# tzjtatata/Myriad

Measured on AMD Instinct MI355X. Metric: images/sec fine-tune step (Vicuna-7B + LoRA-style adapters, 224px), higher is better.
Workload: dtype bf16

## Files before the change

include/myriad_hip.h:

```cpp
#ifndef MYRIAD_HIP_H
#define MYRIAD_HIP_H
#include <stdint.h>

#ifdef __cplusplus
extern "C" {
#endif

typedef struct ihipStream_t* mh_stream_t;

#define MH_OK 0
#define MH_ERR_ARG (-1)
#define MH_ERR_LAUNCH (-2)
#define MH_ERR_UNSUPPORTED (-3)

#define MH_GEMM_OUT_F32 1
#define MH_GEMM_GELU 2
#define MH_GEMM_REGSTAGE 4

int mh_gemm_bf16_nt(const void* A, int lda, const void* B, int ldb, void* C, int ldc, int M, int N, int K,
                    const float* bias, const float* residual, int ldr, int flags, float alpha, mh_stream_t s);

int mh_gemm_plan(int M, int N, int K, int flags, int* kernel, int* splits);

int mh_prof_start(int capacity, mh_stream_t s);
// ... 242 lines not shown
                                   const int* kv_len, const int* live, const float* cos_tab, const float* sin_tab, void* out,
                                   long ldo, float* partials, long partials_floats, int B, int H, int D, int T_cap, int chunk,
                                   float scale, mh_stream_t s);
int mh_patchify_nchw(const float* img, void* out, int B, int C, int H, int W, int P, int Kpad, mh_stream_t s);
int mh_scatter_rows_f32(const float* src, const int* rows, float* dst, long ldd, long n, int D, int accumulate,
                        mh_stream_t s);
int mh_cast_f32_to_bf16(const float* x, void* y, long n, mh_stream_t s);
int mh_cast_bf16_to_f32(const void* x, float* y, long n, mh_stream_t s);
int mh_transpose_to_bf16(const void* in, int in_is_f32, long ldi, void* out, long ldo, int R, int C, mh_stream_t s);
long mh_refresh_bf16_pair_desc_bytes(void);
long mh_refresh_bf16_pair_pack(void* host_table, int index, long first_tile, const float* src, void* dst, long ld_dst,
                               void* dst_t, long ld_t, int R, int C);
int mh_refresh_bf16_pair(const void* dev_table, int n_desc, long total_tiles, mh_stream_t s);
int mh_colsum_f32(const float* in, long ld, float* out, long R, int C, mh_stream_t s);
int mh_scale_f32(float* x, float a, long n, mh_stream_t s);

int mh_adamw_step(float* p, const float* g, float* m, float* v, void* shadow_bf16, long n, double lr, double beta1,
                  double beta2, double eps, double weight_decay, int step, double grad_scale, mh_stream_t s);

int mh_patch_blend_u8(void* out, const void* src, const void* masks, const void* ops, const int* hs, const int* ws,
                      int n_ops, int B, int H, int W, void* union_mask, const void* patches, mh_stream_t s);
int mh_patch_label(const void* dest, const void* out, const void* union_mask, void* sums_ws, void* lm_ws, float* label,
                   const double* factor, int B, int H, int W, int mode, int tol, double k, double x0, mh_stream_t s);
int mh_patch_resize_u8(const void* src, int image, int H, int W, int sy, int sx, int sh, int sw, const int* xi, const int* xw,
                       const int* yi, const int* yw, void* out, int h, int w, mh_stream_t s);
long mh_patch_poisson_ws_doubles(int h, int w);
int mh_patch_poisson_u8(void* out, int image, int H, int W, const void* patch, int hp, int wp, const void* pms,
                        const void* eroded, int y0s, int x0s, int dy0, int dx0, int h, int w, const double* Sh, const double* cy,
                        const double* Sw, const double* cx, double* ws, int mixed, mh_stream_t s);

int mh_adamw_gated(float* p, const float* g, float* m, float* v, long n, double lr, double beta1, double beta2, double eps,
                   double weight_decay, double grad_scale, const float* used, const int* steps, mh_stream_t s);
int mh_adamw_bump(const float* used, int* steps, int n, mh_stream_t s);

int mh_l2norm_rows(const float* x, long ldx, void* y_bf16, float* y_f32, long ldy, int M, int D, float eps, mh_stream_t s);
int mh_pair_logits(const float* p, long ldp, const float* text, float* out, long rows, int rows_per_batch, int C, float scale,
                   mh_stream_t s);
int mh_zs_accumulate(const float* logits, float* mask_acc, float* map_acc, int B, int h, int S, float w, mh_stream_t s);
int mh_rowmax_skip(const float* scores, long lds, float* acc, long rows, int cols, int period, float w, mh_stream_t s);
int mh_bilinear_ac(const float* in, float* out, int B, int h, int w, int H, int W, int one_minus, mh_stream_t s);

typedef struct mh_ctx mh_ctx;
int mh_ctx_create(mh_ctx** out);
int mh_ctx_destroy(mh_ctx* ctx);
int mh_ctx_set_workspace(mh_ctx* ctx, mh_stream_t stream, void* ptr, long bytes);
int mh_ctx_make_current(mh_ctx* ctx);
int mh_ctx_comm_id(void* id128);
int mh_ctx_comm_init(mh_ctx* ctx, const void* id128, int rank, int world);
int mh_ctx_world(const mh_ctx* ctx);
int mh_allreduce_start(mh_ctx* ctx, float* buf, long n, mh_stream_t producer);
#define MH_DT_F32 0
#define MH_DT_BF16 1
int mh_allreduce_start_dt(mh_ctx* ctx, void* buf, long n, int dt, mh_stream_t producer);
int mh_reduce_scatter_start(mh_ctx* ctx, const void* send, void* recv, long n_per_rank, int dt, mh_stream_t producer);
int mh_allgather_start(mh_ctx* ctx, const void* send, void* recv, long n_per_rank, int dt, mh_stream_t producer);
int mh_allreduce_wait(mh_ctx* ctx, mh_stream_t consumer);

const char* mh_version(void);
int mh_target_arch(void);

int mh_set_option(const char* name, int value);
int mh_get_option(const char* name);
int mh_bf16_round_check(const float* x, void* hw, void* hw_pk, void* sw, long n, mh_stream_t s);

int mh_image_resize_crop_norm(const void* img, int H, int W, long row_stride, const int* kh, const int* bh, int ksz_h,
                              const int* kv, const int* bv, int ksz_v, int crop_y0, int crop_x0, int out_h, int out_w, int y0,
// ... 8 lines not shown
```

myriad_amd/csrc/optim.hip:

```cpp
#include "common.h"

__global__ void adamw_kernel(float* __restrict__ p, const float* __restrict__ g, float* __restrict__ m,
                             float* __restrict__ v, bf16_t* __restrict__ shadow, long n4, float lr, float beta1,
                             float beta2, float omb1, float omb2, float eps, float wd, float bc1, float bc2_sqrt,
                             float gscale) {
  for (long it = blockIdx.x * (long)blockDim.x + threadIdx.x; it < n4; it += (long)gridDim.x * blockDim.x) {
    float4_t pp = *reinterpret_cast<const float4_t*>(p + it * 4);
    const float4_t gg = *reinterpret_cast<const float4_t*>(g + it * 4);
    float4_t mm = *reinterpret_cast<const float4_t*>(m + it * 4);
    float4_t vv = *reinterpret_cast<const float4_t*>(v + it * 4);
#pragma unroll
    for (int e = 0; e < 4; ++e) {
      const float gr = gg[e] * gscale;
      pp[e] *= (1.f - lr * wd);
      mm[e] = beta1 * mm[e] + omb1 * gr;
      vv[e] = beta2 * vv[e] + omb2 * gr * gr;
      const float denom = sqrtf(vv[e]) / bc2_sqrt + eps;
      pp[e] -= (lr / bc1) * (mm[e] / denom);
    }
    *reinterpret_cast<float4_t*>(p + it * 4) = pp;
    *reinterpret_cast<float4_t*>(m + it * 4) = mm;
    *reinterpret_cast<float4_t*>(v + it * 4) = vv;
    if (shadow) {
      uint2 pk;
      pk.x = pack_bf2(pp[0], pp[1]);
      pk.y = pack_bf2(pp[2], pp[3]);
      *reinterpret_cast<uint2*>(shadow + it * 4) = pk;
    }
  }
}

extern "C" int mh_adamw_step(float* p, const float* g, float* m, float* v, void* shadow_bf16, long n, double lr,
                             double beta1, double beta2, double eps, double weight_decay, int step, double grad_scale,
                             hipStream_t stream) {
  if (n <= 0) return MH_OK;
  if (n % 4 || step < 1) return MH_ERR_ARG;
  const float bc1 = (float)(1.0 - pow(beta1, (double)step));
  const float bc2s = (float)sqrt(1.0 - pow(beta2, (double)step));
  const float omb1 = (float)(1.0 - beta1), omb2 = (float)(1.0 - beta2);
  long grid = (n / 4 + 255) / 256;
  if (grid > 256 * 16) grid = 256 * 16;
  hipLaunchKernelGGL(adamw_kernel, dim3((int)grid), dim3(256), 0, stream, p, g, m, v, (bf16_t*)shadow_bf16, n / 4,
                     (float)lr, (float)beta1, (float)beta2, omb1, omb2, (float)eps, (float)weight_decay, bc1, bc2s,
                     (float)grad_scale);
  MH_CHECK_LAUNCH();
  return MH_OK;
}

__global__ void adamw_gated_kernel(float* __restrict__ p, const float* __restrict__ g, float* __restrict__ m,
                                   float* __restrict__ v, long n4, float lr, double beta1_d, double beta2_d, float eps,
                                   float wd, float gscale, const float* __restrict__ used, const int* __restrict__ steps) {
  if (*used <= 0.f) return;
  const double st = (double)(*steps + 1);
  const float bc1 = (float)(1.0 - pow(beta1_d, st));
  const float bc2_sqrt = (float)sqrt(1.0 - pow(beta2_d, st));
  const float omb1 = (float)(1.0 - beta1_d), omb2 = (float)(1.0 - beta2_d);
  const float beta1 = (float)beta1_d, beta2 = (float)beta2_d;
  for (long it = blockIdx.x * (long)blockDim.x + threadIdx.x; it < n4; it += (long)gridDim.x * blockDim.x) {
    float4_t pp = *reinterpret_cast<const float4_t*>(p + it * 4);
    const float4_t gg = *reinterpret_cast<const float4_t*>(g + it * 4);
    float4_t mm = *reinterpret_cast<const float4_t*>(m + it * 4);
    float4_t vv = *reinterpret_cast<const float4_t*>(v + it * 4);
#pragma unroll
    for (int e = 0; e < 4; ++e) {
      const float gr = gg[e] * gscale;
      pp[e] *= (1.f - lr * wd);
      mm[e] = beta1 * mm[e] + omb1 * gr;
      vv[e] = beta2 * vv[e] + omb2 * gr * gr;
      const float denom = sqrtf(vv[e]) / bc2_sqrt + eps;
      pp[e] -= (lr / bc1) * (mm[e] / denom);
    }
    *reinterpret_cast<float4_t*>(p + it * 4) = pp;
    *reinterpret_cast<float4_t*>(m + it * 4) = mm;
    *reinterpret_cast<float4_t*>(v + it * 4) = vv;
  }
}
__global__ void adamw_bump_kernel(const float* __restrict__ used, int* __restrict__ steps, int n) {
  const int i = blockIdx.x * blockDim.x + threadIdx.x;
  if (i < n && used[i] > 0.f) steps[i] += 1;
}

extern "C" int mh_adamw_gated(float* p, const float* g, float* m, float* v, long n, double lr, double beta1, double beta2,
                              double eps, double weight_decay, double grad_scale, const float* used, const int* steps,
                              hipStream_t stream) {
  if (n <= 0) return MH_OK;
  if (n % 4 || !used || !steps) return MH_ERR_ARG;
  long grid = (n / 4 + 255) / 256;
  if (grid > 256 * 16) grid = 256 * 16;
  hipLaunchKernelGGL(adamw_gated_kernel, dim3((int)grid), dim3(256), 0, stream, p, g, m, v, n / 4, (float)lr, beta1, beta2,
                     (float)eps, (float)weight_decay, (float)grad_scale, used, steps);
  MH_CHECK_LAUNCH();
  return MH_OK;
}
extern "C" int mh_adamw_bump(const float* used, int* steps, int n, hipStream_t stream) {
  if (n <= 0) return MH_OK;
  hipLaunchKernelGGL(adamw_bump_kernel, dim3((n + 63) / 64), dim3(64), 0, stream, used, steps, n);
  MH_CHECK_LAUNCH();
  return MH_OK;
}
```

myriad_amd/myriad.py:

```python
from __future__ import annotations

import numbers
import os
import random
from collections import OrderedDict
from typing import Dict, List, Optional, Tuple

import torch
import torch.nn as nn

from . import _lib, ops
from .eva_vit import EvaViTHIP
from .llama import LlamaHIP
from .networks import LoraAdaptor, VENet, from_reference_layout, to_reference_layout, ve_param_specs
from .qformer import QFormerHIP, qformer_param_specs
from .registry import registry

BF16, F32 = torch.bfloat16, torch.float32


def uses_weight_decay(name: str, ndim: int) -> bool:
    return not (ndim < 2 or "bias" in name or "ln" in name or "bn" in name)


# ... 67 lines not shown
            o, n = self.offsets[name]
            self.p[name] = self.flat_p[o:o + n].view(ishape)
            self.g[name] = self.flat_g[o:o + n].view(ishape)
            self.ref_shape[name] = rshape
        self.step = 0
        self.version = 0

    def n_params(self) -> int:
        return sum(n for _, n in self.offsets.values())

    def mark_used(self, used_modules) -> None:
        if not self.modules:
            return
        flags = torch.tensor([1.0 if m in used_modules else 0.0 for m in self.modules], dtype=F32)
        self.used.copy_(ops.h2d(flags, self.dev))

    def module_steps(self) -> Dict[str, int]:
        st = self.steps_dev.cpu().tolist()
        return {m: int(st[i]) for i, m in enumerate(self.modules)}

    def set_module_steps(self, steps: Dict[str, int]) -> None:
        host = torch.tensor([int(steps.get(m, 0)) for m in self.modules] or [0], dtype=torch.int32)
        self.steps_dev.copy_(host.to(self.dev))

    def module_range(self, module: str, decays: bool = True):
        if module not in self.modules:
            return None
        mi = self.modules.index(module)
        for m2, a, b, d in self.ranges:
            if m2 == mi and d == decays:
                return a, b
        return None

    def adamw_module(self, module: str, lr: float, weight_decay: float = 0.05, beta2: float = 0.999) -> None:
        mi = self.modules.index(module)
        self.version += 1
        for m2, a, b, decays in self.ranges:
            if m2 == mi:
                ops.adamw_gated(self.flat_p[a:b], self.flat_g[a:b], self.flat_m[a:b], self.flat_v[a:b], lr,
                                weight_decay if decays else 0.0, self.used[mi:mi + 1], self.steps_dev[mi:mi + 1], beta2=beta2)

    def adamw_pieces(self, pieces, lr: float, weight_decay: float = 0.05, beta2: float = 0.999, grad_scale: float = 1.0) -> None:
        self.version += 1
        for mi, a0, b0, decays in self.ranges:
            for lo, hi in pieces:
                a, b = max(a0, lo), min(b0, hi)
                if a < b:
                    ops.adamw_gated(self.flat_p[a:b], self.flat_g[a:b], self.flat_m[a:b], self.flat_v[a:b], lr,
                                    weight_decay if decays else 0.0, self.used[mi:mi + 1], self.steps_dev[mi:mi + 1], beta2=beta2,
                                    grad_scale=grad_scale)

    def adamw_step(self, lr: float, weight_decay: float = 0.05, beta2: float = 0.999, grad_scale: float = 1.0, shard=None,
                   skip=(), exclude=()):
        self.step += 1
        self.version += 1
        pieces = None
        if shard is not None:
            pieces = [tuple(shard)] if isinstance(shard[0], int) else [tuple(p) for p in shard]
            if sum(hi - lo for lo, hi in pieces) < self.total:
                self.moments_complete = False
        skip_idx = {self.modules.index(m) for m in skip if m in self.modules}
        for mi, a0, b0, decays in self.ranges:
            if mi in skip_idx:
                continue
            for lo, hi in (pieces if pieces is not None else [(a0, b0)]):
                a, b = max(a0, lo), min(b0, hi)
                if a >= b:
                    continue
                todo = [(a, b)]
                for ex_lo, ex_hi in exclude:
                    todo = [q for (x, y) in todo for q in ((x, min(y, ex_lo)), (max(x, ex_hi), y)) if q[0] < q[1]]
                for a, b in todo:
                    ops.adamw_gated(self.flat_p[a:b], self.flat_g[a:b], self.flat_m[a:b], self.flat_v[a:b], lr,
# ... 107 lines not shown
            if name in lora_init and name not in weights:
                src = lora_init[name]
            elif name in weights:
                src = weights[name]
            else:
                src = init_trainable(name, rshape)
            self.store.p[name].copy_(from_reference_layout(src.to(self._dev, F32), ishape))
            prm = nn.Parameter(self.store.p[name], requires_grad=True)
            prm.grad = self.store.g[name]
            self._params[name] = prm
            self._register_dotted(name, prm)
        if self.arch == "myriad":
            self.adaptor = LoraAdaptor(self.store.p, self.store.g)
            self.ve_tok = VENet("VETokenizer.", 5, self.Dl, self.store.p, self.store.g, self._dev)
            self.ve_ins = VENet("VEInstructor.", 1, self.Dq, self.store.p, self.store.g, self._dev)
        if self.use_lora:
            self.lora = LoraQV(len(self.llama.layers), self.Dl, int(cfg.get("lora_r", 8)),
                               float(cfg.get("lora_alpha", 16)), float(cfg.get("lora_dropout", 0.05)),
                               self.store.p, self.store.g, self._dev)
            self.lora.base_seed = int(cfg.get("lora_dropout_seed", torch.initial_seed())) & ((1 << 31) - 1)
            self.llama.attach_lora(self.lora)
        if self.train_qformer:
            self.query_tokens_f32 = self.store.p["query_tokens"]
            self.qformer.bind_trainable(self.store, need_denc=self.arch == "myriad" or self.train_vit)
        if self.train_vit:
            self.ln_w, self.ln_b = self.store.p["ln_vision.weight"], self.store.p["ln_vision.bias"]
            self.vit.bind_trainable(self.store, need_backward=need_bwd)
        self._pending_update = None
        self._vit_stream, self._vit_prefetched = None, None
        self._vit_graphs, self._vit_seen, self._vit_rest = {}, {}, None
        self._vit_split = int(os.environ.get("MYRIAD_VIT_SPLIT", "22"))
        self._vit_graph_on = os.environ.get("MYRIAD_VIT_GRAPH", "1") != "0"
        self._leaf_aside = os.environ.get("MYRIAD_LEAF_STREAM", "1") != "0"
        self._anchor = torch.zeros((), device=self._dev, requires_grad=True)
        self._ctx = None
        self._has_grads, self._bwd_gscale, self._bwd_prev = False, 1.0, None
        self._accum_count = 0
        self._bridge_used = set()

    def _register_dotted(self, name: str, prm: nn.Parameter):
        mod = self
        parts = name.split(".")
        for part in parts[:-1]:
            if not hasattr(mod, part) or not isinstance(getattr(mod, part), nn.Module):
                setattr(mod, part, nn.Module())
            mod = getattr(mod, part)
        mod.register_parameter(parts[-1], prm)

    @property
    def device(self):
        return self._dev

    def to(self, *args, **kwargs):
        dev = args[0] if args else kwargs.get("device", self._dev)
        if isinstance(dev, (str, torch.device)):
            d = torch.device(dev)
            if d.type != self._dev.type or (d.index is not None and d.index != self._dev.index):
                raise RuntimeError(f"{type(self).__name__} lives on {self._dev}; build it there (cfg.device; no CPU path exists)")
        return self

    def before_evaluation(self, **kwargs):
        pass

    def state_dict(self, *a, **k):
        self.finish_update()
        out = OrderedDict()
# ... 279 lines not shown
        self._acc_head = head
        fg = self.store.flat_g_comm
        if not accumulate:
            prev = None
        elif head is None:
            prev = fg.clone()
        else:
            prev = (fg[:head[0]].clone(), fg[head[1]:].clone())
        zeroed, self._g_zeroed = getattr(self, "_g_zeroed", None), None
        if zeroed is not None and not accumulate:
            torch.cuda.current_stream().wait_event(zeroed)
        elif head is None:
            fg.zero_()
        else:
            fg[:head[0]].zero_()
            fg[head[1]:].zero_()
        used = {"lora"} if self.use_lora else set()
        if self.arch == "myriad":
            used.add("expert_adaptor")
            if c["use_tok"]:
                used.add("VETokenizer")
            if c["use_ins"]:
                used.add("VEInstructor")
        else:
            used.add("llama_proj")
        if self.train_qformer:
            used.add("Qformer")
        if self.train_vit:
            used.update(("visual_encoder", "ln_vision"))
        self.store.mark_used(used)
        self._bridge_used = (self._bridge_used | used) if accumulate else set(used)
        self._bwd_gscale, self._bwd_prev = float(gscale), prev
        self._early_done = set()
        demb = self.llama.backward(defer_lora_join=True)
        self._prefetch_vit_rest()
        B, nq = c["B"], c["nq"]
        (c0, n0) = c["img_slices"][0]
        dimg = torch.empty((B, nq, self.Dl), dtype=F32, device=self._dev)
        ops.copy3d(demb[:, c0:c0 + n0], dimg)
        dimg_b = ops.to_bf16(dimg.view(B * nq, self.Dl))
        if self.arch != "myriad":
            ops.gemm_auto_f32(ops.transpose_to_bf16(dimg_b, 64), ops.transpose_to_bf16(c["qo_b"], 64),
                              self.store.g["llama_proj.weight"])
            self.store.g["llama_proj.bias"].copy_(ops.colsum(dimg.view(B * nq, self.Dl)))
            if self.train_qformer or self.train_vit:
                pwT = ops.transpose_to_bf16(ops.to_bf16(self.store.p["llama_proj.weight"]), 64)
                dqo = ops.gemm(dimg_b, pwT, out_dtype=F32).view(B, nq, self.Dq)
                dq, denc = self.qformer.backward(dqo, wgrads=self.train_qformer, want_denc=self.train_vit)
                if self.train_qformer:
                    self._query_tokens_grad(dq)
                if self.train_vit:
                    dy = self._ln_vision_backward(denc, c)
                    self.vit.backward(dy.view(B, c["N"], self.Dv), grads=self.vit.grad_views)
            if self.llama.lora is not None:
                self.llama.lora.join_wgrads()
            self._finish_backward()
            return
        dqo = ops.gemm(dimg_b, self.proj_wT, out_dtype=F32).view(B, nq, self.Dq)
        if c["use_tok"]:
            (cb, _), (ct, _) = c["img_slices"][1], c["img_slices"][2]
            dbase = torch.empty((B, 9, self.Dl), dtype=F32, device=self._dev)
            ops.copy3d(demb[:, cb:cb + 9], dbase)
            self.store.g["VETokenizer.base_prompts"].view(-1).copy_(ops.colsum(dbase.view(B, 9 * self.Dl)))
            dtok = torch.empty((B, 9, self.Dl), dtype=F32, device=self._dev)
            ops.copy3d(demb[:, ct:ct + 9], dtok)
            aux, main = (self._side_stream("leaf") if self._leaf_aside else torch.cuda.current_stream()), torch.cuda.current_stream()
            aux.wait_stream(main)
            leaf_keep = (dtok, self.ve_tok._saved)
            with torch.cuda.stream(aux):
                self.ve_tok.backward(dtok, accumulate_head=self._acc_head is not None)
                if early_adamw is not None and self._leaf_aside:
                    self.store.adamw_module("VETokenizer", *early_adamw)
                    self._early_done = {"VETokenizer"}
                if early_exchange is not None:
                    self._start_early_exchange(early_exchange)
                leaf_ev = torch.cuda.Event()
                leaf_ev.record()
        else:
            leaf_ev, leaf_keep = None, None
            if early_exchange is not None:
                self._start_early_exchange(early_exchange)
        dq, denc = self.qformer.backward(dqo, wgrads=self.train_qformer)
        if self.train_qformer:
            self._query_tokens_grad(dq)
        ins_ev, ins_keep = None, None
        if c["use_ins"]:
            dins = torch.empty((B, 49, self.Dq), dtype=F32, device=self._dev)
            ops.copy3d(dq[:, self.nq0:], dins)
            if self._leaf_aside and self._dev.type == "cuda" and os.environ.get("MYRIAD_INS_ASIDE", "1") != "0":
                aux, main = self._side_stream("leaf"), torch.cuda.current_stream()
                aux.wait_stream(main)
                ins_keep = (dins, self.ve_ins._saved)
                with torch.cuda.stream(aux):
                    self.ve_ins.backward(dins)
                    ins_ev = torch.cuda.Event()
                    ins_ev.record()
            else:
                self.ve_ins.backward(dins)
        dy = self._ln_vision_backward(denc, c)
        dx = self.adaptor.backward(dy, need_dx=self.train_vit)
        if self.train_vit:
            self.vit.backward(dx.view(B, c["N"], self.Dv), grads=self.vit.grad_views)
        if self.llama.lora is not None:
            self.llama.lora.join_wgrads()
        if leaf_ev is not None:
            torch.cuda.current_stream().wait_event(leaf_ev)
# ... 134 lines not shown
    def _take_prefetched_vit(self, samples):
        if self._vit_rest is not None and self._vit_rest[0] is samples:
            self._prefetch_vit_rest()
        if self._vit_prefetched is None or self._vit_prefetched[0] is not samples:
            return None
        _, out, ev = self._vit_prefetched
        self._vit_prefetched = None
        main = torch.cuda.current_stream()
        main.wait_event(ev)
        out.record_stream(main)
        return out

    def train_step(self, samples, lr: float, weight_decay: float = 0.05, allreduce=None, world: int = 1, dp=None,
                   overlap: bool = True, next_samples=None, accum_grad_iters: int = 1, accum_index=None, beta2: float = 0.999):
        with torch.no_grad():
            vit_out = self._take_prefetched_vit(samples)
            if next_samples is not None:
                self.prefetch_vit(next_samples)
            if self._pending_update is not None and vit_out is not None:
                self.finish_update()
            elif self._pending_update is not None and self.train_vit:
                self.finish_update()
            elif self._pending_update is not None:
                vit_out = self.vit.forward(self._image_of(samples))
                self.finish_update()
            if (self._accum_count == 0 and self._leaf_aside and self._dev.type == "cuda"
                    and os.environ.get("MYRIAD_EARLY_ZERO", "1") != "0"):
                aux, main = self._side_stream("leaf"), torch.cuda.current_stream()
                aux.wait_stream(main)
                with torch.cuda.stream(aux):
                    self.store.flat_g_comm.zero_()
                    self._g_zeroed = torch.cuda.Event()
                    self._g_zeroed.record(aux)
            try:
                loss = self._forward_impl(samples, True, vit_out=vit_out)
            except Exception:
                self._g_zeroed = None
                raise
            accumulate = self._accum_count > 0
            due = accum_update_due(self._accum_count + 1, accum_grad_iters, accum_index)
            early = (lr, weight_decay, beta2) if (due and not accumulate and (dp is None or dp.world == 1) and allreduce is None
                                                  and world == 1 and os.environ.get("MYRIAD_EARLY_ADAMW", "1") != "0") else None
            if dp is not None and dp.world > 1 and self.arch == "myriad" and hasattr(dp, "set_segments"):
                self._dp_segment(dp)
            early_x = None
            if (dp is not None and dp.world > 1 and overlap and due and not accumulate and self.arch == "myriad"
                    and hasattr(dp, "start_part") and os.environ.get("MYRIAD_DP_EARLY", "1") != "0"):
                k = self._dp_segment(dp)
                if k is not None:
                    early_x = (dp, k, (lr, weight_decay, beta2)) if os.environ.get("MYRIAD_DP_EARLY_ADAMW", "1") != "0" else (dp, k)
            self.backward(accumulate=accumulate, early_adamw=early, early_exchange=early_x)
            self._accum_count += 1
            if not due:
                return loss
            self._accum_count = 0
            if dp is not None and dp.world > 1 and overlap:
                dp.start(self.store.flat_g_comm, self.store.total)
                self._pending_update = (dp, lr, weight_decay, beta2)
            else:
                shard = None
                if dp is not None and dp.world > 1:
                    dp.allreduce(self.store.flat_g_comm, self.store.total)
                    shard = self._dp_shards(dp)
                elif allreduce is not None:
                    allreduce(self.store.flat_g_comm)
                    world = max(world, 1)
                self.store.adamw_step(lr, weight_decay, beta2=beta2, grad_scale=1.0 / (dp.world if dp is not None else world),
                                      shard=shard, skip=self._early_done)
                if shard is not None:
                    dp.gather_params(self.store.flat_p)
        return loss

    def _dp_shards(self, dp):
        if getattr(dp, "mode", "allreduce") != "rs_ag":
            return None
        return dp.shards(self.store.total) if hasattr(dp, "shards") else [dp.shard(self.store.total)[:2]]

    def _dp_segment(self, dp):
        if getattr(self, "_dp_seg_of", None) is not None and self._dp_seg_of[0] is dp:
            return self._dp_seg_of[1]
        k = None
        rng = self.store.module_range("VETokenizer", True)
        if rng is not None:
            a, b = ops.round_up(rng[0], 32), rng[1] // 32 * 32
            if b - a >= (1 << 20):
                dp.set_segments(self.store.total, [a, b])
                segs = dp.segments(self.store.total)
                k = segs.index((a, b)) if (a, b) in segs else None
        self._dp_seg_of = (dp, k)
        return k

    def finish_update(self):
        if self._pending_update is not None:
            dp, lr, wd, beta2 = self._pending_update
            self._pending_update = None
            if dp is None:
                self.store.adamw_step(lr, wd, beta2=beta2)
                return
            dp.wait()
            shard = self._dp_shards(dp)
            done = dp.take_early_done() if hasattr(dp, "take_early_done") else set()
            segs = dp.segments(self.store.total) if done else []
            self.store.adamw_step(lr, wd, beta2=beta2, grad_scale=1.0 / dp.world, shard=shard, exclude=[segs[k] for k in done])
# ... 198 lines not shown
```

myriad_amd/networks.py:

```python
from __future__ import annotations

from typing import Dict, List, Optional, Tuple

import torch

from . import ops

BF16, F32 = torch.bfloat16, torch.float32

STEM_CH = [(1, 4), (4, 16), (16, 64), (64, 256), (256, 1024)]
STEM_IDX = (0, 3, 6, 9, 12)


def ve_param_specs(prefix: str, head_out: int, head_k: int) -> List[Tuple[str, Tuple[int, ...], Tuple[int, ...]]]:
    specs = []
    for idx, (ci, co) in zip(STEM_IDX, STEM_CH):
        specs.append((f"{prefix}meta_net.{idx}.weight", (co, 9 * ci), (co, ci, 3, 3)))
        specs.append((f"{prefix}meta_net.{idx}.bias", (co,), (co,)))
    specs.append((f"{prefix}meta_net.15.weight", (head_out, head_k * head_k * 1024), (head_out, 1024, head_k, head_k)))
    specs.append((f"{prefix}meta_net.15.bias", (head_out,), (head_out,)))
    return specs


def from_reference_layout(t: torch.Tensor, internal_shape) -> torch.Tensor:
    if t.dim() == 4 and len(internal_shape) != 4:
        return t.permute(0, 2, 3, 1).reshape(internal_shape).contiguous()
    return t.reshape(internal_shape).contiguous()


def to_reference_layout(t: torch.Tensor, ref_shape) -> torch.Tensor:
    if len(ref_shape) == 4 and t.dim() != 4:
        co, ci, kh, kw = ref_shape
        return t.reshape(co, kh, kw, ci).permute(0, 3, 1, 2).contiguous()
    return t.reshape(ref_shape).contiguous()


class VENet:

    def __init__(self, prefix: str, head_k: int, head_out: int, params: Dict[str, torch.Tensor],
                 grads: Dict[str, torch.Tensor], device):
        self.prefix, self.head_k, self.head_out = prefix, head_k, head_out
        self.p, self.g, self.dev = params, grads, torch.device(device)
        self._saved = None

    def _w(self, idx):
        return self.p[f"{self.prefix}meta_net.{idx}.weight"], self.p[f"{self.prefix}meta_net.{idx}.bias"]

    def forward(self, maps: torch.Tensor, save_for_backward: bool = True) -> torch.Tensor:
        B, _, H, W = maps.shape
        x = ops.to_bf16(maps.contiguous()).view(B, H, W, 1)
        saved = []
        for idx, (ci, co) in zip(STEM_IDX, STEM_CH):
            wm, bias = self._w(idx)
            wp = ops.conv_pack(wm, bias)
            col = ops.im2col(x, 3, 3, 1)
            y = ops.gemm(col, wp, out_dtype=F32)
            saved.append((col, y, wp, H, W, ci, co))
            x = ops.relu_pool_fwd(y, B, H, W, co)
            H, W = H // 2, W // 2
        wm, bias = self._w(15)
        if self.head_k == 1:
            x2 = x.view(B * H * W, 1024)
            wb = ops.to_bf16(wm)
            out = ops.gemm(x2, wb, bias=bias, out_dtype=F32)
            head = (x2, wb, None, True)
            T = H * W
        else:
            k = self.head_k
            T = (H - k + 1) * (W - k + 1)
            if wm.shape[1] % 64 == 0:
                wp = ops.to_bf16(wm)
                col = ops.im2col(x, k, k, 0, bias_col=False)
                out = ops.gemm(col, wp, bias=bias, out_dtype=F32)
                head = (col, wp, (H, W), True)
            else:
                wp = ops.conv_pack(wm, bias)
                col = ops.im2col(x, k, k, 0)
                out = ops.gemm(col, wp, out_dtype=F32)
                head = (col, wp, (H, W), False)
        if save_for_backward:
            self._saved = dict(stem=saved, head=head, B=B)
        return out.view(B, T, self.head_out)

    @property
    def head_accumulates_in_place(self) -> bool:
        return self.head_k != 1 and (self.head_k * self.head_k * 1024) % 64 == 0

    def backward(self, dtokens: torch.Tensor, accumulate_head: bool = False) -> None:
        sv = self._saved
        if sv is None:
            raise RuntimeError("backward() without saved forward")
        B = sv["B"]
        dy32 = dtokens.reshape(-1, self.head_out).contiguous()
        dyb = ops.to_bf16(dy32)
        gw, gb = self.g[f"{self.prefix}meta_net.15.weight"], self.g[f"{self.prefix}meta_net.15.bias"]
        a, wq, hw = sv["head"][:3]
        dyT = ops.transpose_to_bf16(dyb, 64)
        if self.head_k == 1:
            ops.gemm_auto_f32(dyT, ops.transpose_to_bf16(a, 64), gw)
            gb.copy_(ops.colsum(dy32))
            dp = ops.gemm(dyb, ops.transpose_to_bf16(wq, 64), out_dtype=F32)
        else:
            Kpad = wq.shape[1]
            if sv["head"][3]:
                if accumulate_head:
                    ops.gemm(dyT, ops.transpose_to_bf16(a, 64), out=gw, residual=gw)
                else:
                    ops.gemm_auto_f32(dyT, ops.transpose_to_bf16(a, 64), gw)
                gb.copy_(ops.colsum(dy32))
            else:
                dwp = torch.empty((self.head_out, Kpad), dtype=F32, device=self.dev)
                ops.gemm_auto_f32(dyT, ops.transpose_to_bf16(a, 64), dwp)
                ops.conv_unpack_grad(dwp, gw, gb)
            dcol = ops.gemm(dyb, ops.transpose_to_bf16(wq, 64))
            H, W = hw
            dp = ops.col2im(dcol, B, H, W, 1024, self.head_k, self.head_k, 0)
        for li in range(4, -1, -1):
            col, y, wp, H, W, ci, co = sv["stem"][li]
            idx = STEM_IDX[li]
            dy, dyfull = ops.relu_pool_bwd(dp, y, B, H, W, co, pad_cols_to=64)
            dwp = torch.empty((co, wp.shape[1]), dtype=F32, device=self.dev)
            ops.gemm_auto_f32(ops.transpose_to_bf16(dy, 64), ops.transpose_to_bf16(col, 64), dwp)
            ops.conv_unpack_grad(dwp, self.g[f"{self.prefix}meta_net.{idx}.weight"],
                                 self.g[f"{self.prefix}meta_net.{idx}.bias"])
            if li > 0:
                wpT = ops.transpose_to_bf16(wp, 64)
                dcol = ops.gemm(dyfull, wpT)
                dp = ops.col2im(dcol, B, H, W, ci, 3, 3, 1)
        self._saved = None


class LoraAdaptor:

    def __init__(self, params, grads, prefix="expert_adaptor."):
        self.A, self.Bm = params[prefix + "conv1.weight"], params[prefix + "conv2.weight"]
        self.gA, self.gB = grads[prefix + "conv1.weight"], grads[prefix + "conv2.weight"]
        self._saved = None

    def forward(self, x2d: torch.Tensor, save_for_backward=True):
        y, t = ops.lowrank_fwd(x2d, self.A, self.Bm)
        if save_for_backward:
            self._saved = (x2d, t)
        return y

    def backward(self, dy2d: torch.Tensor, need_dx: bool = False):
        x2d, t = self._saved
        dx = ops.lowrank_bwd(dy2d, x2d, t, self.A, self.Bm, self.gA, self.gB, need_dx=need_dx)
# ... 3 lines not shown
```

myriad_amd/ops.py:

```python
from __future__ import annotations

import math
import numbers
from typing import Optional

import os

import torch

from . import _lib

BF16 = torch.bfloat16
F32 = torch.float32

GEMM_OUT_F32 = 1
GEMM_GELU = 2
GEMM_REGSTAGE = 4
GEMM_VARIANT = 0


def _L():
    return _lib.load()


# ... 1213 lines not shown
    return full[:, :C], full


def conv_pack(Wm: torch.Tensor, bias: Optional[torch.Tensor], out=None):
    Cout, K = Wm.shape
    Kpad = round_up(K + 1, 64)
    if out is None:
        out = torch.empty((Cout, Kpad), dtype=BF16, device=Wm.device)
    _lib.check(_L().mh_conv_pack_weight(_p(Wm), _p(bias), _p(out), Cout, K, Kpad, _s()), "mh_conv_pack_weight")
    return out


def conv_unpack_grad(dWp: torch.Tensor, dW: torch.Tensor, db: Optional[torch.Tensor]):
    Cout, Kpad = dWp.shape
    K = dW.shape[1]
    _lib.check(_L().mh_conv_unpack_grad(_p(dWp), _p(dW), _p(db), Cout, K, Kpad, _s()), "mh_conv_unpack_grad")


def adamw_step(p, g, m, v, lr, wd, step, beta1=0.9, beta2=0.999, eps=1e-8, grad_scale=1.0, shadow=None):
    _lib.check(_L().mh_adamw_step(_p(p), _p(g), _p(m), _p(v), _p(shadow), p.numel(), float(lr), float(beta1),
                                  float(beta2), float(eps), float(wd), int(step), float(grad_scale), _s()),
               "mh_adamw_step")


def adamw_gated(p, g, m, v, lr, wd, used: torch.Tensor, steps: torch.Tensor, beta1=0.9, beta2=0.999, eps=1e-8, grad_scale=1.0):
    _lib.check(_L().mh_adamw_gated(_p(p), _p(g), _p(m), _p(v), p.numel(), float(lr), float(beta1), float(beta2), float(eps),
                                   float(wd), float(grad_scale), _p(used), _p(steps), _s()), "mh_adamw_gated")


def adamw_bump(used: torch.Tensor, steps: torch.Tensor):
    _lib.check(_L().mh_adamw_bump(_p(used), _p(steps), steps.numel(), _s()), "mh_adamw_bump")


def l2norm_rows(x: torch.Tensor, want_bf16: bool = True, want_f32: bool = False, eps: float = 1e-12):
    _chk2d(x, F32, "l2norm_rows.x")
    M, D = x.shape
    yb = torch.empty((M, D), dtype=BF16, device=x.device) if want_bf16 else None
    yf = torch.empty((M, D), dtype=F32, device=x.device) if want_f32 else None
    _lib.check(_L().mh_l2norm_rows(_p(x), x.stride(0), _p(yb), _p(yf), D, M, D, float(eps), _s()), "mh_l2norm_rows")
    return yb, yf


def pair_logits(p: torch.Tensor, text: torch.Tensor, rows_per_batch: int, scale: float = 100.0):
    _chk2d(p, F32, "pair_logits.p")
    rows, C = p.shape
    out = torch.empty((rows, 2), dtype=F32, device=p.device)
    _lib.check(_L().mh_pair_logits(_p(p), p.stride(0), _p(text.contiguous()), _p(out), rows, rows_per_batch, C, float(scale),
                                   _s()), "mh_pair_logits")
    return out


def zs_accumulate(logits: torch.Tensor, mask_acc: torch.Tensor, map_acc: torch.Tensor, w: float):
    B, h, S = mask_acc.shape[0], mask_acc.shape[-1], map_acc.shape[-1]
    _lib.check(_L().mh_zs_accumulate(_p(logits), _p(mask_acc), _p(map_acc), B, h, S, float(w), _s()), "mh_zs_accumulate")


def rowmax_skip(scores: torch.Tensor, acc: torch.Tensor, period: int, w: float):
    rows, cols = scores.shape
    _lib.check(_L().mh_rowmax_skip(_p(scores), scores.stride(0), _p(acc), rows, cols, period, float(w), _s()), "mh_rowmax_skip")


def bilinear_ac(x: torch.Tensor, H: int, W: int, one_minus: bool = False):
    B, h, w = x.shape
    out = torch.empty((B, H, W), dtype=F32, device=x.device)
    _lib.check(_L().mh_bilinear_ac(_p(x.contiguous()), _p(out), B, h, w, H, W, int(one_minus), _s()), "mh_bilinear_ac")
    return out
# ... 32 lines not shown
```

Measured before the change: 203.4.

## Fuse VETokenizer head weight-gradient GEMM with AdamW and keep bf16 weight copies

Adds a HIP kernel that computes the head weight gradient tile by tile with MFMA, applies the gated AdamW update in registers, and writes the fp32 param, moments, gradient, a bf16 copy and a transposed bf16 copy in one pass. The backward path defers the head wgrad GEMM and the optimizer calls this kernel for the head's slice, splitting the other ranges around it. The kept bf16 copies are stamped with a version key so the next forward and backward can reuse them instead of re-converting and re-transposing the weight. This saves a separate GEMM, the AdamW pass over the head and the conversion kernels, at the cost of extra buffers, staleness-tracking logic and a naive unpipelined MFMA loop that reads K directly from global memory.

New measurement: 203.3. About the same (-0.1%).

```diff
diff --git a/include/myriad_hip.h b/include/myriad_hip.h
--- a/include/myriad_hip.h
+++ b/include/myriad_hip.h
@@ -298,6 +298,10 @@
 int mh_adamw_gated(float* p, const float* g, float* m, float* v, long n, double lr, double beta1, double beta2, double eps,
                    double weight_decay, double grad_scale, const float* used, const int* steps, mh_stream_t s);
 int mh_adamw_bump(const float* used, int* steps, int n, mh_stream_t s);
+int mh_adamw_head_fused_supported(int R, int C, int Kp, long ldw, long ldt);
+int mh_adamw_head_fused(float* p, float* m, float* v, float* g, const void* dyT, const void* colT, void* w_bf16, long ldw,
+                        void* wT_bf16, long ldt, int R, int C, int Kp, double lr, double beta1, double beta2, double eps,
+                        double weight_decay, double grad_scale, const float* used, const int* steps, mh_stream_t s);
 
 int mh_l2norm_rows(const float* x, long ldx, void* y_bf16, float* y_f32, long ldy, int M, int D, float eps, mh_stream_t s);
 int mh_pair_logits(const float* p, long ldp, const float* text, float* out, long rows, int rows_per_batch, int C, float scale,
diff --git a/myriad_amd/csrc/optim.hip b/myriad_amd/csrc/optim.hip
--- a/myriad_amd/csrc/optim.hip
+++ b/myriad_amd/csrc/optim.hip
@@ -47,29 +47,43 @@
   return MH_OK;
 }
 
+struct AdamwCoef { float bc1, bc2_sqrt, omb1, omb2, beta1, beta2; };
+__device__ __forceinline__ AdamwCoef adamw_coef(double beta1_d, double beta2_d, int steps_done) {
+  const double st = (double)(steps_done + 1);
+  AdamwCoef k;
+  k.bc1 = (float)(1.0 - pow(beta1_d, st));
+  k.bc2_sqrt = (float)sqrt(1.0 - pow(beta2_d, st));
+  k.omb1 = (float)(1.0 - beta1_d);
+  k.omb2 = (float)(1.0 - beta2_d);
+  k.beta1 = (float)beta1_d;
+  k.beta2 = (float)beta2_d;
+  return k;
+}
+__device__ __forceinline__ void adamw_update4(float4_t& pp, const float4_t gg, float4_t& mm, float4_t& vv, const AdamwCoef k,
+                                              float lr, float eps, float wd, float gscale) {
+#pragma clang fp contract(off)
+  const float decay = __builtin_fmaf(-lr, wd, 1.f);
+  const float step = lr / k.bc1;
+#pragma unroll
+  for (int e = 0; e < 4; ++e) {
+    const float gr = gg[e] * gscale;
+    mm[e] = __builtin_fmaf(mm[e], k.beta1, gr * k.omb1);
+    vv[e] = __builtin_fmaf(vv[e], k.beta2, gr * (gr * k.omb2));
+    const float denom = sqrtf(vv[e]) / k.bc2_sqrt + eps;
+    pp[e] = __builtin_fmaf(decay, pp[e], -(step * (mm[e] / denom)));
+  }
+}
 __global__ void adamw_gated_kernel(float* __restrict__ p, const float* __restrict__ g, float* __restrict__ m,
                                    float* __restrict__ v, long n4, float lr, double beta1_d, double beta2_d, float eps,
                                    float wd, float gscale, const float* __restrict__ used, const int* __restrict__ steps) {
   if (*used <= 0.f) return;
-  const double st = (double)(*steps + 1);
-  const float bc1 = (float)(1.0 - pow(beta1_d, st));
-  const float bc2_sqrt = (float)sqrt(1.0 - pow(beta2_d, st));
-  const float omb1 = (float)(1.0 - beta1_d), omb2 = (float)(1.0 - beta2_d);
-  const float beta1 = (float)beta1_d, beta2 = (float)beta2_d;
+  const AdamwCoef k = adamw_coef(beta1_d, beta2_d, *steps);
   for (long it = blockIdx.x * (long)blockDim.x + threadIdx.x; it < n4; it += (long)gridDim.x * blockDim.x) {
     float4_t pp = *reinterpret_cast<const float4_t*>(p + it * 4);
     const float4_t gg = *reinterpret_cast<const float4_t*>(g + it * 4);
     float4_t mm = *reinterpret_cast<const float4_t*>(m + it * 4);
     float4_t vv = *reinterpret_cast<const float4_t*>(v + it * 4);
-#pragma unroll
-    for (int e = 0; e < 4; ++e) {
-      const float gr = gg[e] * gscale;
-      pp[e] *= (1.f - lr * wd);
-      mm[e] = beta1 * mm[e] + omb1 * gr;
-      vv[e] = beta2 * vv[e] + omb2 * gr * gr;
-      const float denom = sqrtf(vv[e]) / bc2_sqrt + eps;
-      pp[e] -= (lr / bc1) * (mm[e] / denom);
-    }
+    adamw_update4(pp, gg, mm, vv, k, lr, eps, wd, gscale);
     *reinterpret_cast<float4_t*>(p + it * 4) = pp;
     *reinterpret_cast<float4_t*>(m + it * 4) = mm;
     *reinterpret_cast<float4_t*>(v + it * 4) = vv;
@@ -98,3 +112,130 @@
   MH_CHECK_LAUNCH();
   return MH_OK;
 }
+
+#define HF_T 64
+#define HF_TR 64
+#define HF_GLD 68
+
+__global__ __launch_bounds__(256) void adamw_head_fused_kernel(
+    float* __restrict__ p, float* __restrict__ m, float* __restrict__ v, float* __restrict__ gout,
+    const bf16_t* __restrict__ dyT, const bf16_t* __restrict__ colT, bf16_t* __restrict__ w, bf16_t* __restrict__ wT, int R, int C,
+    int Kp, long ldw, long ldt, int tiles_r, float lr, double beta1_d, double beta2_d, float eps, float wd, float gscale,
+    const float* __restrict__ used, const int* __restrict__ steps) {
+  constexpr int TR = HF_TR;
+  constexpr int NIT = TR / 32;
+  constexpr int TLD = TR / 2 + 1;
+  constexpr int RF = TR / 16;
+  constexpr int JL = TR / 4;
+  __shared__ __attribute__((aligned(16))) float G[TR][HF_GLD];
+  __shared__ unsigned T[HF_T][TLD];
+  if (*used <= 0.f) return;
+  const int t = threadIdx.x;
+  const int r0 = ((int)blockIdx.x % tiles_r) * TR, c0 = ((int)blockIdx.x / tiles_r) * HF_T;
+  const int sg = t & 15, sc = c0 + 4 * sg;
+
+  float4_t pp[NIT][2], mm[NIT][2], vv[NIT][2];
+#pragma unroll
+  for (int it = 0; it < NIT; ++it)
+#pragma unroll
+    for (int h = 0; h < 2; ++h) {
+      const int r = r0 + 2 * ((t >> 4) + 16 * it) + h;
+      if (r < R) {
+        const long o = (long)r * C + sc;
+        pp[it][h] = *reinterpret_cast<const float4_t*>(p + o);
+        mm[it][h] = *reinterpret_cast<const float4_t*>(m + o);
+        vv[it][h] = *reinterpret_cast<const float4_t*>(v + o);
+      }
+    }
+
+  {
+    const int lane = t & 63, wave = t >> 6;
+    const int lr_ = lane & 15, lg = lane >> 4;
+    const int fr = wave % RF, fc = (wave / RF) * RF;
+    int ra = r0 + fr * 16 + lr_;
+    ra = ra < R ? ra : R - 1;
+    const bf16_t* ga = dyT + (long)ra * Kp + lg * 8;
+    const bf16_t* gb = colT + (long)(c0 + fc * 16 + lr_) * Kp + lg * 8;
+    float4_t acc[RF];
+#pragma unroll
+    for (int j = 0; j < RF; ++j) acc[j] = (float4_t){0.f, 0.f, 0.f, 0.f};
+    for (int k0 = 0; k0 < Kp; k0 += 32) {
+      short8_t bfr[RF];
+#pragma unroll
+      for (int j = 0; j < RF; ++j) bfr[j] = *reinterpret_cast<const short8_t*>(gb + (long)j * 16 * Kp + k0);
+      const short8_t af = *reinterpret_cast<const short8_t*>(ga + k0);
+#pragma unroll
+      for (int j = 0; j < RF; ++j) acc[j] = __builtin_amdgcn_mfma_f32_16x16x32_bf16(bfr[j], af, acc[j], 0, 0, 0);
+    }
+#pragma unroll
+    for (int j = 0; j < RF; ++j) *reinterpret_cast<float4_t*>(&G[fr * 16 + lr_][(fc + j) * 16 + lg * 4]) = acc[j];
+  }
+  __syncthreads();
+
+  const AdamwCoef k = adamw_coef(beta1_d, beta2_d, *steps);
+#pragma unroll
+  for (int it = 0; it < NIT; ++it) {
+    const int pr = (t >> 4) + 16 * it;
+#pragma unroll
+    for (int h = 0; h < 2; ++h) {
+      const int r = r0 + 2 * pr + h;
+      if (r < R) {
+        const float4_t gg = *reinterpret_cast<const float4_t*>(&G[2 * pr + h][4 * sg]);
+        adamw_update4(pp[it][h], gg, mm[it][h], vv[it][h], k, lr, eps, wd, gscale);
+        const long o = (long)r * C + sc;
+        *reinterpret_cast<float4_t*>(p + o) = pp[it][h];
+        *reinterpret_cast<float4_t*>(m + o) = mm[it][h];
+        *reinterpret_cast<float4_t*>(v + o) = vv[it][h];
+        *reinterpret_cast<float4_t*>(gout + o) = gg;
+        uint2 pk;
+        pk.x = pack_bf2(pp[it][h][0], pp[it][h][1]);
+        pk.y = pack_bf2(pp[it][h][2], pp[it][h][3]);
+        *reinterpret_cast<uint2*>(w + (long)r * ldw + sc) = pk;
+      } else {
+        pp[it][h] = (float4_t){0.f, 0.f, 0.f, 0.f};
+      }
+    }
+#pragma unroll
+    for (int e = 0; e < 4; ++e) T[4 * sg + e][pr] = pack_bf2(pp[it][0][e], pp[it][1][e]);
+  }
+  __syncthreads();
+  {
+    const int j = t % JL, r = r0 + 4 * j;
+    if (r < R) {
+#pragma unroll
+      for (int it = 0; it < HF_T / (256 / JL); ++it) {
+        const int ci = t / JL + (256 / JL) * it;
+        uint2 pk;
+        pk.x = T[ci][2 * j];
+        pk.y = T[ci][2 * j + 1];
+        *reinterpret_cast<uint2*>(wT + (long)(c0 + ci) * ldt + r) = pk;
+      }
+    }
+  }
+}
+
+extern "C" int mh_adamw_head_fused_supported(int R, int C, int Kp, long ldw, long ldt) {
+  if (R <= 0 || C <= 0 || Kp <= 0 || R % 4 || C % 64 || Kp % 64) return MH_ERR_UNSUPPORTED;
+  if (ldw < C || ldw % 4 || ldt < R || ldt % 4) return MH_ERR_UNSUPPORTED;
+  if (((long)(R + HF_TR - 1) / HF_TR) * (C / HF_T) > 0x7fffffffL) return MH_ERR_UNSUPPORTED;
+  return MH_OK;
+}
+
+extern "C" int mh_adamw_head_fused(float* p, float* m, float* v, float* g, const void* dyT, const void* colT, void* w_bf16,
+                                   long ldw, void* wT_bf16, long ldt, int R, int C, int Kp, double lr, double beta1, double beta2,
+                                   double eps, double weight_decay, double grad_scale, const float* used, const int* steps,
+                                   hipStream_t stream) {
+  if (!p || !m || !v || !g || !dyT || !colT || !w_bf16 || !wT_bf16 || !used || !steps) return MH_ERR_ARG;
+  const int rc = mh_adamw_head_fused_supported(R, C, Kp, ldw, ldt);
+  if (rc) return rc;
+  if ((((uintptr_t)p | (uintptr_t)m | (uintptr_t)v | (uintptr_t)g | (uintptr_t)dyT | (uintptr_t)colT) & 15) ||
+      (((uintptr_t)w_bf16 | (uintptr_t)wT_bf16) & 7))
+    return MH_ERR_UNSUPPORTED;
+  const int tiles_r = (R + HF_TR - 1) / HF_TR;
+  const long tiles = (long)tiles_r * (C / HF_T);
+  hipLaunchKernelGGL(adamw_head_fused_kernel, dim3((unsigned)tiles), dim3(256), 0, stream, p, m, v, g, (const bf16_t*)dyT,
+                     (const bf16_t*)colT, (bf16_t*)w_bf16, (bf16_t*)wT_bf16, R, C, Kp, ldw, ldt, tiles_r, (float)lr, beta1, beta2,
+                     (float)eps, (float)weight_decay, (float)grad_scale, used, steps);
+  MH_CHECK_LAUNCH();
+  return MH_OK;
+}
diff --git a/myriad_amd/myriad.py b/myriad_amd/myriad.py
--- a/myriad_amd/myriad.py
+++ b/myriad_amd/myriad.py
@@ -123,13 +123,37 @@
                 return a, b
         return None
 
-    def adamw_module(self, module: str, lr: float, weight_decay: float = 0.05, beta2: float = 0.999) -> None:
+    def content_key(self):
+        return (self.version, self.flat_p._version)
+
+    def adamw_module(self, module: str, lr: float, weight_decay: float = 0.05, beta2: float = 0.999, fused_head=None) -> None:
         mi = self.modules.index(module)
         self.version += 1
+        cut = None
+        if fused_head is not None:
+            name, net = fused_head
+            o, n = self.offsets[name]
+            cut = (o, o + n)
         for m2, a, b, decays in self.ranges:
-            if m2 == mi:
-                ops.adamw_gated(self.flat_p[a:b], self.flat_g[a:b], self.flat_m[a:b], self.flat_v[a:b], lr,
-                                weight_decay if decays else 0.0, self.used[mi:mi + 1], self.steps_dev[mi:mi + 1], beta2=beta2)
+            if m2 != mi:
+                continue
+            pieces = [(a, b)]
+            if cut is not None and a <= cut[0] and cut[1] <= b:
+                pieces = [(a, cut[0]), cut, (cut[1], b)]
+            for lo, hi in pieces:
+                if lo >= hi:
+                    continue
+                wd = weight_decay if decays else 0.0
+                if (lo, hi) == cut:
+                    shape = self.p[name].shape
+                    net.fused_head_update(self.p[name], self.g[name], self.flat_m[lo:hi].view(shape), self.flat_v[lo:hi].view(shape),
+                                          lr, wd, self.used[mi:mi + 1], self.steps_dev[mi:mi + 1], beta2=beta2)
+                    cut = None
+                else:
+                    ops.adamw_gated(self.flat_p[lo:hi], self.flat_g[lo:hi], self.flat_m[lo:hi], self.flat_v[lo:hi], lr, wd,
+                                    self.used[mi:mi + 1], self.steps_dev[mi:mi + 1], beta2=beta2)
+        if fused_head is not None and cut is not None:
+            raise RuntimeError(f"adamw_module: {fused_head[0]} lies in no range of {module}")
 
     def adamw_pieces(self, pieces, lr: float, weight_decay: float = 0.05, beta2: float = 0.999, grad_scale: float = 1.0) -> None:
         self.version += 1
@@ -303,6 +327,8 @@
         self._vit_split = int(os.environ.get("MYRIAD_VIT_SPLIT", "22"))
         self._vit_graph_on = os.environ.get("MYRIAD_VIT_GRAPH", "1") != "0"
         self._leaf_aside = os.environ.get("MYRIAD_LEAF_STREAM", "1") != "0"
+        self._head_fused_on = os.environ.get("MYRIAD_HEAD_FUSED", "1") != "0"
+        self._head_fused_ran, self._step_used_tok = False, False
         self._anchor = torch.zeros((), device=self._dev, requires_grad=True)
         self._ctx = None
         self._has_grads, self._bwd_gscale, self._bwd_prev = False, 1.0, None
@@ -648,6 +674,7 @@
         self._bridge_used = (self._bridge_used | used) if accumulate else set(used)
         self._bwd_gscale, self._bwd_prev = float(gscale), prev
         self._early_done = set()
+        self._head_fused_ran, self._step_used_tok = False, bool(self.arch == "myriad" and c["use_tok"])
         demb = self.llama.backward(defer_lora_join=True)
         self._prefetch_vit_rest()
         B, nq = c["B"], c["nq"]
@@ -683,11 +710,15 @@
             aux, main = (self._side_stream("leaf") if self._leaf_aside else torch.cuda.current_stream()), torch.cuda.current_stream()
             aux.wait_stream(main)
             leaf_keep = (dtok, self.ve_tok._saved)
+            fuse_head = (early_adamw is not None and self._leaf_aside and self._head_fused_on and self._acc_head is None
+                         and not accumulate and float(gscale) == 1.0 and self.ve_tok.head_fusable(B * 9))
             with torch.cuda.stream(aux):
-                self.ve_tok.backward(dtok, accumulate_head=self._acc_head is not None)
+                self.ve_tok.backward(dtok, accumulate_head=self._acc_head is not None, defer_head_wgrad=fuse_head)
                 if early_adamw is not None and self._leaf_aside:
-                    self.store.adamw_module("VETokenizer", *early_adamw)
+                    self.store.adamw_module("VETokenizer", *early_adamw,
+                                            fused_head=("VETokenizer.meta_net.15.weight", self.ve_tok) if fuse_head else None)
                     self._early_done = {"VETokenizer"}
+                    self._head_fused_ran = fuse_head
                 if early_exchange is not None:
                     self._start_early_exchange(early_exchange)
                 leaf_ev = torch.cuda.Event()
@@ -888,15 +919,23 @@
                     self.store.flat_g_comm.zero_()
                     self._g_zeroed = torch.cuda.Event()
                     self._g_zeroed.record(aux)
+            accumulate = self._accum_count > 0
+            due = accum_update_due(self._accum_count + 1, accum_grad_iters, accum_index)
+            early = (lr, weight_decay, beta2) if (due and not accumulate and (dp is None or dp.world == 1) and allreduce is None
+                                                  and world == 1 and os.environ.get("MYRIAD_EARLY_ADAMW", "1") != "0") else None
+            tok = self.ve_tok if self.arch == "myriad" else None
+            copies_current = bool(tok is not None and early is not None and self._head_fused_on
+                                  and tok.head_copies.current(self.store.content_key()))
             try:
+                if tok is not None:
+                    tok.use_kept = copies_current
                 loss = self._forward_impl(samples, True, vit_out=vit_out)
             except Exception:
                 self._g_zeroed = None
                 raise
-            accumulate = self._accum_count > 0
-            due = accum_update_due(self._accum_count + 1, accum_grad_iters, accum_index)
-            early = (lr, weight_decay, beta2) if (due and not accumulate and (dp is None or dp.world == 1) and allreduce is None
-                                                  and world == 1 and os.environ.get("MYRIAD_EARLY_ADAMW", "1") != "0") else None
+            finally:
+                if tok is not None:
+                    tok.use_kept = False
             if dp is not None and dp.world > 1 and self.arch == "myriad" and hasattr(dp, "set_segments"):
                 self._dp_segment(dp)
             early_x = None
@@ -925,6 +964,9 @@
                                       shard=shard, skip=self._early_done)
                 if shard is not None:
                     dp.gather_params(self.store.flat_p)
+                if tok is not None and early is not None:
+                    if self._head_fused_ran or (copies_current and not self._step_used_tok):
+                        tok.head_copies.stamp(self.store.content_key())
         return loss
 
     def _dp_shards(self, dp):
diff --git a/myriad_amd/networks.py b/myriad_amd/networks.py
--- a/myriad_amd/networks.py
+++ b/myriad_amd/networks.py
@@ -35,6 +35,25 @@
     return t.reshape(ref_shape).contiguous()
 
 
+class HeadCopyState:
+
+    def __init__(self):
+        self._key = None
+        self.stamps = 0
+
+    def stamp(self, key) -> None:
+        if key is None:
+            raise ValueError("HeadCopyState.stamp: a key is required")
+        self._key = key
+        self.stamps += 1
+
+    def invalidate(self) -> None:
+        self._key = None
+
+    def current(self, key) -> bool:
+        return self._key is not None and key is not None and self._key == key
+
+
 class VENet:
 
     def __init__(self, prefix: str, head_k: int, head_out: int, params: Dict[str, torch.Tensor],
@@ -42,6 +61,12 @@
         self.prefix, self.head_k, self.head_out = prefix, head_k, head_out
         self.p, self.g, self.dev = params, grads, torch.device(device)
         self._saved = None
+        self.head_copies = HeadCopyState()
+        self.w_bf16: Optional[torch.Tensor] = None
+        self.wT_bf16: Optional[torch.Tensor] = None
+        self.use_kept = False
+        self.head_forwards_kept, self.head_forwards_rebuilt = 0, 0
+        self._head_operands = None
 
     def _w(self, idx):
         return self.p[f"{self.prefix}meta_net.{idx}.weight"], self.p[f"{self.prefix}meta_net.{idx}.bias"]
@@ -69,10 +94,16 @@
             k = self.head_k
             T = (H - k + 1) * (W - k + 1)
             if wm.shape[1] % 64 == 0:
-                wp = ops.to_bf16(wm)
+                kept = self.use_kept and self.w_bf16 is not None
+                if kept:
+                    wp = self.w_bf16
+                    self.head_forwards_kept += 1
+                else:
+                    wp = ops.to_bf16(wm)
+                    self.head_forwards_rebuilt += 1
                 col = ops.im2col(x, k, k, 0, bias_col=False)
                 out = ops.gemm(col, wp, bias=bias, out_dtype=F32)
-                head = (col, wp, (H, W), True)
+                head = (col, wp, (H, W), True, kept)
             else:
                 wp = ops.conv_pack(wm, bias)
                 col = ops.im2col(x, k, k, 0)
@@ -86,7 +117,25 @@
     def head_accumulates_in_place(self) -> bool:
         return self.head_k != 1 and (self.head_k * self.head_k * 1024) % 64 == 0
 
-    def backward(self, dtokens: torch.Tensor, accumulate_head: bool = False) -> None:
+    def head_fusable(self, n_rows: int) -> bool:
+        if not self.head_accumulates_in_place:
+            return False
+        return ops.adamw_head_fused_supported(self.head_out, self.head_k * self.head_k * 1024, ops.round_up(n_rows, 64))
+
+    def fused_head_update(self, p, g, m, v, lr, wd, used, steps, beta2=0.999) -> None:
+        if self._head_operands is None:
+            raise RuntimeError("fused_head_update() without a backward(defer_head_wgrad=True)")
+        dyT, colT = self._head_operands
+        self._head_operands = None
+        R, C = p.shape
+        if self.w_bf16 is None:
+            self.w_bf16 = torch.zeros((R, C), dtype=BF16, device=self.dev)
+            self.wT_bf16 = torch.zeros((C, ops.round_up(R, 64)), dtype=BF16, device=self.dev)
+        self.head_copies.invalidate()
+        if not ops.adamw_head_fused(p, g, m, v, dyT, colT, self.w_bf16, self.wT_bf16, lr, wd, used, steps, beta2=beta2):
+            raise RuntimeError("the fused head update refused a head that head_fusable() accepted: its weight gradient is lost")
+
+    def backward(self, dtokens: torch.Tensor, accumulate_head: bool = False, defer_head_wgrad: bool = False) -> None:
         sv = self._saved
         if sv is None:
             raise RuntimeError("backward() without saved forward")
@@ -96,6 +145,8 @@
         gw, gb = self.g[f"{self.prefix}meta_net.15.weight"], self.g[f"{self.prefix}meta_net.15.bias"]
         a, wq, hw = sv["head"][:3]
         dyT = ops.transpose_to_bf16(dyb, 64)
+        if defer_head_wgrad and (accumulate_head or not self.head_accumulates_in_place):
+            raise ValueError("defer_head_wgrad: only for a head_fusable() head outside an accumulation window")
         if self.head_k == 1:
             ops.gemm_auto_f32(dyT, ops.transpose_to_bf16(a, 64), gw)
             gb.copy_(ops.colsum(dy32))
@@ -105,6 +156,8 @@
             if sv["head"][3]:
                 if accumulate_head:
                     ops.gemm(dyT, ops.transpose_to_bf16(a, 64), out=gw, residual=gw)
+                elif defer_head_wgrad:
+                    self._head_operands = (dyT, ops.transpose_to_bf16(a, 64))
                 else:
                     ops.gemm_auto_f32(dyT, ops.transpose_to_bf16(a, 64), gw)
                 gb.copy_(ops.colsum(dy32))
@@ -112,7 +165,8 @@
                 dwp = torch.empty((self.head_out, Kpad), dtype=F32, device=self.dev)
                 ops.gemm_auto_f32(dyT, ops.transpose_to_bf16(a, 64), dwp)
                 ops.conv_unpack_grad(dwp, gw, gb)
-            dcol = ops.gemm(dyb, ops.transpose_to_bf16(wq, 64))
+            wqT = self.wT_bf16 if len(sv["head"]) > 4 and sv["head"][4] else ops.transpose_to_bf16(wq, 64)
+            dcol = ops.gemm(dyb, wqT)
             H, W = hw
             dp = ops.col2im(dcol, B, H, W, 1024, self.head_k, self.head_k, 0)
         for li in range(4, -1, -1):
diff --git a/myriad_amd/ops.py b/myriad_amd/ops.py
--- a/myriad_amd/ops.py
+++ b/myriad_amd/ops.py
@@ -1269,6 +1269,36 @@
     _lib.check(_L().mh_adamw_bump(_p(used), _p(steps), steps.numel(), _s()), "mh_adamw_bump")
 
 
+def adamw_head_fused_supported(R: int, C: int, Kp: int, ldw: Optional[int] = None, ldt: Optional[int] = None) -> bool:
+    ldw = C if ldw is None else ldw
+    ldt = round_up(R, 64) if ldt is None else ldt
+    return _L().mh_adamw_head_fused_supported(int(R), int(C), int(Kp), int(ldw), int(ldt)) == 0
+
+
+def adamw_head_fused(p, g, m, v, dyT: torch.Tensor, colT: torch.Tensor, w_bf16: torch.Tensor, wT_bf16: torch.Tensor, lr, wd,
+                     used: torch.Tensor, steps: torch.Tensor, beta1=0.9, beta2=0.999, eps=1e-8, grad_scale=1.0) -> bool:
+    R, C = p.shape
+    for t, name in ((p, "p"), (g, "g"), (m, "m"), (v, "v")):
+        if t.dtype != F32 or tuple(t.shape) != (R, C) or not t.is_contiguous():
+            raise _lib.MyriadHipError(f"adamw_head_fused.{name}: need a contiguous f32 [{R}, {C}]")
+    _chk2d(dyT, BF16, "adamw_head_fused.dyT")
+    _chk2d(colT, BF16, "adamw_head_fused.colT")
+    _chk2d(w_bf16, BF16, "adamw_head_fused.w_bf16")
+    _chk2d(wT_bf16, BF16, "adamw_head_fused.wT_bf16")
+    Kp = dyT.shape[1]
+    if dyT.shape[0] != R or tuple(colT.shape) != (C, Kp) or not dyT.is_contiguous() or not colT.is_contiguous():
+        raise _lib.MyriadHipError(f"adamw_head_fused: operands must be dense dyT [{R}, Kp] and colT [{C}, Kp]")
+    if w_bf16.shape[0] < R or w_bf16.shape[1] < C or wT_bf16.shape[0] < C or wT_bf16.shape[1] < R:
+        raise _lib.MyriadHipError(f"adamw_head_fused: copies must be at least [{R}, {C}] and [{C}, {R}]")
+    rc = _L().mh_adamw_head_fused(_p(p), _p(m), _p(v), _p(g), _p(dyT), _p(colT), _p(w_bf16), w_bf16.stride(0), _p(wT_bf16),
+                                  wT_bf16.stride(0), R, C, Kp, float(lr), float(beta1), float(beta2), float(eps), float(wd),
+                                  float(grad_scale), _p(used), _p(steps), _s())
+    if rc == -3:
+        return False
+    _lib.check(rc, f"mh_adamw_head_fused R={R} C={C} Kp={Kp}")
+    return True
+
+
 def l2norm_rows(x: torch.Tensor, want_bf16: bool = True, want_f32: bool = False, eps: float = 1e-12):
     _chk2d(x, F32, "l2norm_rows.x")
     M, D = x.shape
```
